# piotrmwojcik/GI-GS

Measured on AMD Instinct MI355X. Metric: train-step renders/sec (fwd+bwd, G-buffer+indirect) at 800x800; PSNR vs the CPU oracle, higher is better.
Workload: dtype f32; 1 GPU; C2 (configs[1] TensoIR lego stand-in): 300k surface Gaussians, 800x800, SH deg 2, GI step=16 start=8 delta=0.0625; P=300000, N=640000, M=9, hip_graphs=on, fused_glue=on, gi_march=proj, rasterizer=whole step = 2 hand-captured hipGraphs (fwd, bwd), asynchronous binning

## Files before the change

gi-gs_amd/csrc/api.hip:

```cpp
#include <cstdarg>
#include <cstdio>
#include <cstdlib>
#include <cstring>
#include <map>
#include <algorithm>
#include <new>
#include <mutex>
#include <vector>

#include "../../include/gigs_hip.h"
#include "gigs_common.h"

namespace {

thread_local char g_err[512] = "";

int fail(int code, const char* fmt, ...) {
  va_list ap;
  va_start(ap, fmt);
  vsnprintf(g_err, sizeof(g_err), fmt, ap);
  va_end(ap);
  return code;
}

// ... 38 lines not shown
  uint32_t step = msb;
  while (step > 1) {
    step /= 2;
    if (n >> msb) msb += step;
    else msb -= step;
  }
  if (n >> msb) msb++;
  return msb;
}

enum Stage {
  kPreprocess = 0, kScan, kDuplicate, kSort, kRanges, kBlendFwd, kBlendBwd, kPreprocessBwd,
  kDepthToNormal, kSsao, kSsr, kMedian, kBilateral, kMedianBwd, kShadeFwd, kShadeBwd,
  kCubemapFwd, kCubemapBwd, kGbufferPost, kLossFwd, kLossBwd, kL1SsimFwd, kL1SsimBwd, kTvFwd, kTvBwd,
  kMaskedL1, kAdam, kDensifyStats, kGatherRows, kDist2, kActivateFwd, kActivateBwd, kNumStages
};
const char* kStageNames[kNumStages] = {
  "preprocess_fwd", "scan", "duplicate", "sort", "tile_ranges", "blend_fwd", "blend_bwd",
  "preprocess_bwd", "depth_to_normal", "ssao", "ssr", "median3x3", "bilateral3x3",
  "median3x3_bwd", "shade_fwd", "shade_bwd", "cubemap_fwd", "cubemap_bwd", "gbuffer_post",
  "stage2_loss_fwd", "stage2_loss_bwd", "l1_ssim_fwd", "l1_ssim_bwd", "tv_loss_fwd", "tv_loss_bwd", "masked_l1",
  "adam_step", "densify_stats", "gather_rows", "dist2", "activate_fwd", "activate_bwd"};

int env_int(const char* name, int dflt) {
  const char* e = getenv(name);
  return (e && e[0]) ? atoi(e) : dflt;
}
gigs::Options options_from_env() {
  gigs::Options o;
  const char* b = getenv("GIGS_BINNING");
  o.binning_legacy = (b && strcmp(b, "legacy") == 0) ? 1 : 0;
  o.bucket_max_mean = env_int("GIGS_BUCKET_MAX_MEAN", gigs::kBucketMaxMeanList);
  const char* ll = getenv("GIGS_LONG_LISTS");
  o.long_lists = (ll && ll[0]) ? (ll[0] == '1' ? 1 : 0) : -1;
  o.bucket_target = std::max(256, env_int("GIGS_BUCKET_TARGET", 1536));
  o.bin_bands = std::max(0, env_int("GIGS_BIN_BANDS", 0));
  o.blend_cull = env_int("GIGS_BLEND_CULL", 1) != 0;
  o.pre_bwd_sh_skip = env_int("GIGS_PRE_BWD_SH_SKIP", 1) != 0;
  o.gi_march = 4;
  if (const char* e = getenv("GIGS_GI_MARCH")) {
    static const char* names[] = {"exact", "hoist", "hoist_fma", "proj_nr", "proj"};
    for (int i = 0; i < 5; i++)
      if (strcmp(e, names[i]) == 0) o.gi_march = i;
  }
  o.gi_cert = env_int("GIGS_GI_CERT", 1) != 0;
  o.gi_interleave = env_int("GIGS_GI_INTERLEAVE", 1) != 0;
  o.gi_tile_log2w = env_int("GIGS_GI_TILE_LOG2W", 3);
  if (o.gi_tile_log2w < 0 || o.gi_tile_log2w > 6) o.gi_tile_log2w = 3;
  o.gi_zero_rays = env_int("GIGS_GI_ZERO_RAYS", 0) != 0;
  o.spec_max8 = env_int("GIGS_SPEC_MAX8", 128);
  o.spec_max16 = env_int("GIGS_SPEC_MAX16", 1500);
  o.shade_lds_floats = env_int("GIGS_SHADE_LDS_FLOATS", 30 * 1024);
  o.shade_bwd_blocks = std::max(0, env_int("GIGS_SHADE_BWD_BLOCKS", 0));
  return o;
}
const gigs::Ctx& ctx_of(const gigs_ctx* c) { return c ? *reinterpret_cast<const gigs::Ctx*>(c) : gigs::default_ctx(); }

struct ProfRec { int stage; hipEvent_t a, b; };
std::mutex g_prof_mu;
bool g_prof_on = false;
std::vector<ProfRec> g_prof_recs;
std::vector<hipEvent_t> g_prof_pool;

hipEvent_t prof_event() {
  if (!g_prof_pool.empty()) {
    hipEvent_t e = g_prof_pool.back();
    g_prof_pool.pop_back();
    return e;
  }
  hipEvent_t e;
  hipEventCreate(&e);
  return e;
}

struct StageScope {
  hipStream_t s;
  int stage;
  bool on;
  hipEvent_t a, b;
  StageScope(int stage_, hipStream_t s_) : s(s_), stage(stage_), on(false) {
    std::lock_guard<std::mutex> lk(g_prof_mu);
    if (!g_prof_on) return;
    on = true;
    a = prof_event();
    b = prof_event();
    hipEventRecord(a, s);
  }
  ~StageScope() {
    if (!on) return;
    hipEventRecord(b, s);
    std::lock_guard<std::mutex> lk(g_prof_mu);
    g_prof_recs.push_back({stage, a, b});
  }
};

}

namespace gigs {
const Options& default_options() {
  static const Options o = options_from_env();
  return o;
}
const Ctx& default_ctx() {
  static const Ctx c = {default_options(), 0u, nullptr, nullptr, 0, nullptr, nullptr};
  return c;
}
// ... 21 lines not shown
  const size_t N = (size_t)width * height;
  const size_t T = (size_t)((width + GIGS_BLOCK_X - 1) / GIGS_BLOCK_X) * ((height + GIGS_BLOCK_Y - 1) / GIGS_BLOCK_Y);
  return gigs::required_bytes<gigs::ImageState>(N, T);
}
size_t gigs_required_binning(int R) {
  if (R < 0) { fail(GIGS_ERR_INVALID, "R < 0"); return 0; }
  return gigs::required_bytes<gigs::BinningState>((size_t)R, sort_size_cached(R));
}

long long gigs_geom_offset(int P, int which) {
  char* base = nullptr;
  char* p = base;
  gigs::GeomState g = gigs::GeomState::fromChunk(p, (size_t)P, 0);
  const void* ptrs[] = {g.depths, g.pos_view, g.means2D, g.cov3D, g.conic_opacity, g.rgb,
                        g.clamped, g.tiles_touched, g.point_offsets, g.internal_radii, g.brec, g.grec};
  if (which < 0 || which >= (int)(sizeof(ptrs) / sizeof(ptrs[0]))) return -1;
  return (long long)((const char*)ptrs[which] - base);
}
long long gigs_binning_offset(int R, int which) {
  char* base = nullptr;
  char* p = base;
  gigs::BinningState b = gigs::BinningState::fromChunk(p, (size_t)R, 0);
  const void* ptrs[] = {b.keys_unsorted, b.values_unsorted, b.keys, b.point_list, b.hit_mask};
  if (which < 0 || which >= 5) return -1;
  return (long long)((const char*)ptrs[which] - base);
}
long long gigs_image_offset(int width, int height, int which) {
  const size_t N = (size_t)width * height;
  const size_t T = (size_t)((width + GIGS_BLOCK_X - 1) / GIGS_BLOCK_X) * ((height + GIGS_BLOCK_Y - 1) / GIGS_BLOCK_Y);
  char* base = nullptr;
  char* p = base;
  gigs::ImageState s = gigs::ImageState::fromChunk(p, N, T);
  const void* ptrs[] = {s.final_T, s.n_contrib, s.ranges, s.tile_order};
  if (which < 0 || which >= 4) return -1;
  return (long long)((const char*)ptrs[which] - base);
}

gigs_ctx* gigs_ctx_create(void) {
  gigs::Ctx* c = new (std::nothrow) gigs::Ctx(gigs::default_ctx());
  if (!c) fail(GIGS_ERR_ALLOC, "gigs_ctx_create: out of host memory");
  return reinterpret_cast<gigs_ctx*>(c);
}
void gigs_ctx_destroy(gigs_ctx* ctx) { delete reinterpret_cast<gigs::Ctx*>(ctx); }

int gigs_ctx_get_options(const gigs_ctx* ctx, gigs_options* out) {
  if (!out || out->struct_bytes < (int)sizeof(gigs_options)) return fail(GIGS_ERR_INVALID, "gigs_ctx_get_options: set struct_bytes = sizeof(gigs_options)");
  const gigs::Options& o = ctx_of(ctx).opt;
  out->struct_bytes = (int)sizeof(gigs_options);
  out->binning_legacy = o.binning_legacy; out->bucket_max_mean = o.bucket_max_mean; out->long_lists = o.long_lists;
  out->bucket_target = o.bucket_target; out->bin_bands = o.bin_bands; out->blend_cull = o.blend_cull; out->pre_bwd_sh_skip = o.pre_bwd_sh_skip;
  out->gi_march = o.gi_march; out->gi_cert = o.gi_cert; out->gi_interleave = o.gi_interleave;
  out->gi_tile_log2w = o.gi_tile_log2w; out->gi_zero_rays = o.gi_zero_rays; out->spec_max8 = o.spec_max8;
  out->spec_max16 = o.spec_max16; out->shade_lds_floats = o.shade_lds_floats; out->shade_bwd_blocks = o.shade_bwd_blocks;
  return 0;
}
int gigs_ctx_set_options(gigs_ctx* ctx, const gigs_options* in) {
  if (!ctx) return fail(GIGS_ERR_INVALID, "gigs_ctx_set_options: the default context is immutable, create one");
  if (!in || in->struct_bytes < (int)sizeof(gigs_options)) return fail(GIGS_ERR_INVALID, "gigs_ctx_set_options: set struct_bytes = sizeof(gigs_options)");
  if (in->gi_march < 0 || in->gi_march > 4) return fail(GIGS_ERR_INVALID, "gi_march must be 0..4");
  if (in->gi_tile_log2w < 0 || in->gi_tile_log2w > 6) return fail(GIGS_ERR_INVALID, "gi_tile_log2w must be 0..6");
  if (in->long_lists < -1 || in->long_lists > 1) return fail(GIGS_ERR_INVALID, "long_lists must be -1, 0 or 1");
  if (in->bucket_target < 256 || in->bucket_max_mean < 0 || in->bin_bands < 0 || in->bin_bands > 64)
    return fail(GIGS_ERR_INVALID, "bucket_target >= 256, bucket_max_mean >= 0, 0 <= bin_bands <= 64");
  if (in->spec_max8 < 0 || in->spec_max16 < in->spec_max8) return fail(GIGS_ERR_INVALID, "0 <= spec_max8 <= spec_max16");
  if (in->shade_lds_floats < 0 || in->shade_bwd_blocks < 0) return fail(GIGS_ERR_INVALID, "shade_lds_floats, shade_bwd_blocks >= 0");
  gigs::Options& o = reinterpret_cast<gigs::Ctx*>(ctx)->opt;
  o.binning_legacy = in->binning_legacy != 0; o.bucket_max_mean = in->bucket_max_mean; o.long_lists = in->long_lists;
  o.bucket_target = in->bucket_target; o.bin_bands = in->bin_bands; o.blend_cull = in->blend_cull != 0; o.pre_bwd_sh_skip = in->pre_bwd_sh_skip != 0;
  o.gi_march = in->gi_march; o.gi_cert = in->gi_cert != 0; o.gi_interleave = in->gi_interleave != 0;
  o.gi_tile_log2w = in->gi_tile_log2w; o.gi_zero_rays = in->gi_zero_rays != 0; o.spec_max8 = in->spec_max8;
  o.spec_max16 = in->spec_max16; o.shade_lds_floats = in->shade_lds_floats; o.shade_bwd_blocks = in->shade_bwd_blocks;
  return 0;
}
int gigs_ctx_set_reuse_binning(gigs_ctx* ctx, int on) {
  if (!ctx) return fail(GIGS_ERR_INVALID, "gigs_ctx_set_reuse_binning: the default context is immutable, create one");
  reinterpret_cast<gigs::Ctx*>(ctx)->reuse_binning = on != 0;
  return 0;
}
int gigs_ctx_set_split_sh(gigs_ctx* ctx, const float* sh_rest) {
  if (!ctx) return fail(GIGS_ERR_INVALID, "gigs_ctx_set_split_sh: the default context is immutable, create one");
  reinterpret_cast<gigs::Ctx*>(ctx)->sh_rest = sh_rest;
  return 0;
}
int gigs_ctx_set_materials_only(gigs_ctx* ctx, void* violations) {
  if (!ctx) return fail(GIGS_ERR_INVALID, "gigs_ctx_set_materials_only: the default context is immutable, create one");
  reinterpret_cast<gigs::Ctx*>(ctx)->materials_only = reinterpret_cast<unsigned*>(violations);
  return 0;
}
int gigs_ctx_set_blend_begin_event(gigs_ctx* ctx, void* hip_event) {
  if (!ctx) return fail(GIGS_ERR_INVALID, "gigs_ctx_set_blend_begin_event: the default context is immutable, create one");
  reinterpret_cast<gigs::Ctx*>(ctx)->blend_begin_event = hip_event;
  return 0;
}

__global__ void __launch_bounds__(64) stream_delay_kernel(unsigned ticks) {
  const unsigned long long t0 = wall_clock64();
  while (wall_clock64() - t0 < (unsigned long long)ticks) __builtin_amdgcn_s_sleep(8);
}

int gigs_stream_delay(unsigned nanoseconds, void* stream) {
  if (nanoseconds == 0) return 0;
  const unsigned ns = nanoseconds > 1000000u ? 1000000u : nanoseconds;
  hipLaunchKernelGGL(stream_delay_kernel, dim3(1), dim3(64), 0, (hipStream_t)stream, (ns + 9u) / 10u);
  return hipGetLastError() == hipSuccess ? 0 : gigs_internal_fail(GIGS_ERR_HIP, "stream_delay: launch failed");
}

int gigs_ctx_set_async_binning(gigs_ctx* ctx, int r_capacity, unsigned* device_counters) {
  if (!ctx) return fail(GIGS_ERR_INVALID, "gigs_ctx_set_async_binning: the default context is immutable, create one");
  gigs::Ctx* c = reinterpret_cast<gigs::Ctx*>(ctx);
  c->async_capacity = r_capacity > 0 ? (unsigned)r_capacity : 0u;
  c->async_counters = r_capacity > 0 ? device_counters : nullptr;
  return 0;
}

void gigs_profile_begin(void) {
  std::lock_guard<std::mutex> lk(g_prof_mu);
  for (auto& r : g_prof_recs) { g_prof_pool.push_back(r.a); g_prof_pool.push_back(r.b); }
  g_prof_recs.clear();
  g_prof_on = true;
}

int gigs_profile_end(float* total_ms, int* launches, int n) {
  std::vector<ProfRec> recs;
  {
// ... 469 lines not shown
```

gi-gs_amd/csrc/gigs_common.h:

```cpp
#pragma once
#include <hip/hip_runtime.h>
#include <stdint.h>

#define GIGS_BLOCK_X 16
#define GIGS_BLOCK_Y 16
#define GIGS_TILE (GIGS_BLOCK_X * GIGS_BLOCK_Y)
#define GIGS_BREC_F4 5
#define GIGS_GREC 20

namespace gigs {

struct v3 { float x, y, z; };
struct v4 { float x, y, z, w; };

__device__ __forceinline__ v3 operator+(v3 a, v3 b) { return {a.x + b.x, a.y + b.y, a.z + b.z}; }
__device__ __forceinline__ v3 operator-(v3 a, v3 b) { return {a.x - b.x, a.y - b.y, a.z - b.z}; }
__device__ __forceinline__ v3 operator*(v3 a, float s) { return {a.x * s, a.y * s, a.z * s}; }
__device__ __forceinline__ float dot3(v3 a, v3 b) { return a.x * b.x + a.y * b.y + a.z * b.z; }
__device__ __forceinline__ v3 cross3(v3 a, v3 b) {
  return {a.y * b.z - a.z * b.y, a.z * b.x - a.x * b.z, a.x * b.y - a.y * b.x};
}
__device__ __forceinline__ v3 normalize3(v3 v) {
  float inv = 1.0f / sqrtf(dot3(v, v));
  return v * inv;
// ... 131 lines not shown
    carve(chunk, s.n_contrib, N);
    carve(chunk, s.ranges, T);
    carve(chunk, s.tile_order, T);
    carve(chunk, s.bin_hist, (size_t)(kBinGroups + 2) * T);
    carve(chunk, s.bin_counters, 4);
    return s;
  }
};

struct BinningState {
  uint64_t* keys_unsorted;
  uint32_t* values_unsorted;
  uint64_t* keys;
  uint32_t* point_list;
  uint8_t* hit_mask;
  char* sort_space;
  size_t sort_size;
  static BinningState fromChunk(char*& chunk, size_t R, size_t sort_size) {
    BinningState b;
    carve(chunk, b.keys_unsorted, R);
    carve(chunk, b.values_unsorted, R);
    carve(chunk, b.keys, R);
    carve(chunk, b.point_list, R);
    carve(chunk, b.hit_mask, 4 * R);
    b.sort_size = sort_size;
    carve(chunk, b.sort_space, sort_size);
    return b;
  }
};

template <typename S, typename... A>
inline size_t required_bytes(A... a) {
  char* p = nullptr;
  S::fromChunk(p, a...);
  return reinterpret_cast<size_t>(p) + kAlign;
}

struct Options {
  int binning_legacy;
  int bucket_max_mean;
  int long_lists;
  int bucket_target;
  int bin_bands;
  int blend_cull;
  int pre_bwd_sh_skip;
  int gi_march;
  int gi_cert;
  int gi_interleave;
  int gi_tile_log2w;
  int gi_zero_rays;
  int spec_max8, spec_max16;
  int shade_lds_floats;
  int shade_bwd_blocks;
};
struct Ctx {
  Options opt;
  unsigned async_capacity;
  unsigned* async_counters;
  void* blend_begin_event;
  int reuse_binning;
  unsigned* materials_only;
  const float* sh_rest;
};
const Options& default_options();
const Ctx& default_ctx();

struct FwdArgs {
  int P, D, M, W, H;
  unsigned gx, gy;
  float focal_x, focal_y, tan_fovx, tan_fovy, scale_modifier;
  const float *means3D, *shs, *colors_precomp, *opacities, *normal, *albedo, *roughness,
      *metallic, *scales, *rotations, *cov3D_precomp, *viewmatrix, *projmatrix, *cam_pos,
      *background;
  int argmax_depth, inference;
  const float* shs_rest;
};

void launch_preprocess_fwd(const FwdArgs& a, const GeomState& g, int* radii, hipStream_t s);
void launch_zero_words(uint32_t* p, size_t n, hipStream_t s);
void launch_bin_count(int P, const int* radii, unsigned gx, unsigned gy, const GeomState& g, const ImageState& img, hipStream_t s);
void launch_bin_prefix(int P, int T, unsigned capacity, const ImageState& img, unsigned* user_counters, hipStream_t s);
void launch_bin_scatter(int P, const int* radii, unsigned gx, unsigned gy, unsigned capacity, unsigned bands, const GeomState& g,
                        const BinningState& b, const ImageState& img, hipStream_t s);
int launch_bin_sort(int T, int P, bool long_lists, unsigned bucket_target, unsigned capacity, const BinningState& b, const ImageState& img,
                    hipStream_t s);
size_t long_space_bytes(size_t T, size_t R);
void launch_mark_visible(int P, const float* means3D, const float* viewmatrix, uint8_t* present,
                         hipStream_t s);
hipError_t scan_tiles(const GeomState& g, int P, hipStream_t s);
size_t scan_temp_bytes(int P);
size_t sort_temp_bytes(int R);
void launch_duplicate(int P, const int* radii, unsigned gx, unsigned gy, const GeomState& g,
                      const BinningState& b, hipStream_t s);
hipError_t sort_pairs(const BinningState& b, int R, int end_bit, hipStream_t s);
void launch_tile_ranges(int R, const BinningState& b, uint2* ranges, hipStream_t s);
void launch_tile_order(int T, const uint2* ranges, uint32_t* tile_order, hipStream_t s);
void launch_blend_fwd(const FwdArgs& a, const GeomState& g, const BinningState& b,
                      const ImageState& im, float* out_color, float* out_opacity,
                      float* out_depth, float* out_normal, float* out_normal_view, float* out_pos,
                      float* out_albedo, float* out_roughness, float* out_metallic, int cull, size_t hit_stride,
                      hipStream_t s, bool reused_lists = false);

struct BwdArgs {
  int P, D, M, R, W, H;
  unsigned gx, gy;
  float focal_x, focal_y, tan_fovx, tan_fovy, scale_modifier;
// ... 42 lines not shown
```

gi-gs_amd/csrc/pbr.hip:

```cpp
#include <cmath>
#include <cstdlib>
#include <cstring>
#include <map>
#include <mutex>
#include <vector>

#include "gigs_common.h"
#include "pixel_ops.h"

namespace gigs {

__device__ __forceinline__ v3 safe_normalize(v3 v) {
  const float l = sqrtf(v.x * v.x + v.y * v.y + v.z * v.z);
  return l > 0.0f ? v3{v.x / l, v.y / l, v.z / l} : v3{0, 0, 0};
}
__device__ __forceinline__ v3 cube_dir_raw(float fx, float fy, int side) {
  switch (side) {
    case 0: return {1, -fy, -fx};
    case 1: return {-1, -fy, fx};
    case 2: return {fx, 1, fy};
    case 3: return {fx, -1, -fy};
    case 4: return {fx, -fy, 1};
    default: return {-fx, -fy, -1};
  }
// ... 872 lines not shown
cube_taps_export_kernel(int res, int n, const float* __restrict__ dirs, int* __restrict__ idx, float* __restrict__ w) {
  const int i = blockIdx.x * 256 + threadIdx.x;
  if (i >= n) return;
  Taps t;
  const bool ok = cube_taps(res, dirs[3 * (size_t)i], dirs[3 * (size_t)i + 1], dirs[3 * (size_t)i + 2], t);
#pragma unroll
  for (int k = 0; k < 4; k++) {
    const bool use = ok && t.idx[k] >= 0 && t.w[k] != 0.0f;
    idx[4 * (size_t)i + k] = use ? t.idx[k] : -1;
    w[4 * (size_t)i + k] = use ? t.w[k] : 0.0f;
  }
}

__global__ void __launch_bounds__(256)
cube_texture_bwd_gather_kernel(int n_tex, const int* __restrict__ offsets, const int* __restrict__ ent_sample,
                               const float* __restrict__ ent_w, const float* __restrict__ g_out, int n, int planar,
                               float* __restrict__ d_tex, int heavy, int light_blocks, const int* __restrict__ heavy_ids,
                               int n_heavy) {
  auto grad = [&](int s, float& a, float& b, float& c) {
    if (planar) { a = g_out[s]; b = g_out[(size_t)n + s]; c = g_out[2 * (size_t)n + s]; }
    else { a = g_out[3 * (size_t)s]; b = g_out[3 * (size_t)s + 1]; c = g_out[3 * (size_t)s + 2]; }
  };
  if ((int)blockIdx.x < light_blocks) {
    const int t = blockIdx.x * 256 + threadIdx.x;
    if (t >= n_tex) return;
    const int b = offsets[t], e = offsets[t + 1];
    if (e - b > heavy) return;
    float c0 = 0.0f, c1 = 0.0f, c2 = 0.0f;
    for (int k = b; k < e; k++) {
      float g0, g1, g2;
      grad(ent_sample[k], g0, g1, g2);
      const float w = ent_w[k];
      c0 += g0 * w; c1 += g1 * w; c2 += g2 * w;
    }
    d_tex[3 * (size_t)t] = c0; d_tex[3 * (size_t)t + 1] = c1; d_tex[3 * (size_t)t + 2] = c2;
    return;
  }
  const int h = ((int)blockIdx.x - light_blocks) * 4 + (threadIdx.x >> 6);
  if (h >= n_heavy) return;
  const int lane = threadIdx.x & 63;
  const int t = heavy_ids[h];
  const int b = offsets[t], e = offsets[t + 1];
  float c0 = 0.0f, c1 = 0.0f, c2 = 0.0f;
  for (int k = b + lane; k < e; k += 64) {
    float g0, g1, g2;
    grad(ent_sample[k], g0, g1, g2);
    const float w = ent_w[k];
    c0 += g0 * w; c1 += g1 * w; c2 += g2 * w;
  }
  c0 = wave_sum63(c0); c1 = wave_sum63(c1); c2 = wave_sum63(c2);
  if (lane == 63) { d_tex[3 * (size_t)t] = c0; d_tex[3 * (size_t)t + 1] = c1; d_tex[3 * (size_t)t + 2] = c2; }
}

__global__ void __launch_bounds__(kShadeBwdBlock)
shade_bwd_kernel(ShadeArgs A) {
  extern __shared__ __align__(16) float s_lds[];
  for (int i = threadIdx.x; i < A.lds_total; i += kShadeBwdBlock) s_lds[i] = 0.0f;
  __syncthreads();
  const int n_chunks = (A.H * A.W + kShadeBwdBlock - 1) / kShadeBwdBlock;
  for (int chunk = blockIdx.x; chunk < n_chunks; chunk += gridDim.x) {
  const int pg = chunk * kShadeBwdBlock + threadIdx.x;
  const bool live = pg < A.H * A.W;
  const int p = live ? pg : 0;
  ShadePix q;
  shade_pixel(A, p, q);
  float g_dl[3] = {0, 0, 0}, g_sp[3] = {0, 0, 0};
  if (live) {
    const bool mk = A.mask[p] != 0;
    const size_t e = (size_t)p * A.ps, cs = A.cs;
    const float gscale = A.g_scale ? A.g_scale[0] : 1.0f;
    float g_d[3] = {0, 0, 0}, g_s[3] = {0, 0, 0};
    const float pre_d[3] = {q.drgb.x, q.drgb.y, q.drgb.z}, pre_s[3] = {q.srgb.x, q.srgb.y, q.srgb.z};
#pragma unroll
    for (int c = 0; c < 3; c++) {
      float g = (A.g_render && mk) ? A.g_render[e + c * cs] * gscale : 0.0f;
      if (g != 0.0f) {
        float x = pre_d[c] + pre_s[c], d_tone = 1.0f, d_gam = 1.0f;
        if (A.tone) x = aces(x, d_tone);
        const float xc = fminf(fmaxf(x, 0.0f), 1.0f);
        const float d_clamp = (x >= 0.0f && x <= 1.0f) ? 1.0f : 0.0f;
        if (A.gamma) lin2srgb(xc, d_gam);
        g = g * d_gam * d_clamp * d_tone;
      }
      float gd = A.g_diffuse_rgb ? A.g_diffuse_rgb[e + c * cs] : 0.0f;
      float gs = A.g_specular_rgb ? A.g_specular_rgb[e + c * cs] : 0.0f;
      if (A.gamma) {
        float d1, d2;
        lin2srgb(pre_d[c], d1);
        lin2srgb(pre_s[c], d2);
        gd *= d1;
        gs *= d2;
      }
      g_d[c] = g + gd;
      g_s[c] = g + gs;
    }
    const float av[3] = {q.a.x, q.a.y, q.a.z}, dlv[3] = {q.dl.x, q.dl.y, q.dl.z};
    const float spv[3] = {q.sp.x, q.sp.y, q.sp.z}, F0v[3] = {q.F0.x, q.F0.y, q.F0.z};
    const float reflv[3] = {q.refl.x, q.refl.y, q.refl.z};
    const float s0v[3] = {q.s0.x, q.s0.y, q.s0.z}, s1v[3] = {q.s1.x, q.s1.y, q.s1.z};
    float d_alb[3], d_m = 0.0f, d_fgx = 0.0f, d_fgy = 0.0f, d_lvl = 0.0f;
#pragma unroll
    for (int c = 0; c < 3; c++) {
      d_alb[c] = g_d[c] * dlv[c];
      g_dl[c] = g_d[c] * av[c] + (A.g_diffuse_light ? A.g_diffuse_light[e + c * cs] : 0.0f);
      g_sp[c] = g_s[c] * reflv[c];
      const float g_refl = g_s[c] * spv[c];
      const float dF0 = g_refl * q.fgx;
      d_fgx += g_refl * F0v[c];
      d_fgy += g_refl;
      if (A.metallic) {
        d_m += dF0 * (av[c] - 0.04f);
        d_alb[c] += dF0 * q.m;
      }
      if (q.l1 != q.l0) d_lvl += g_sp[c] * (s1v[c] - s0v[c]);
    }
#pragma unroll
    for (int c = 0; c < 3; c++) {
      if (A.g_albedo_mul_a) d_alb[c] += (A.g_albedo_mul_a[e + c * cs] * gscale) * A.g_albedo_mul_b[e + c * cs];
      A.d_albedo[e + c * cs] = d_alb[c];
    }
    float add_r = A.g_roughness_add ? A.g_roughness_add[p] : 0.0f, add_m = A.g_metallic_add ? A.g_metallic_add[p] : 0.0f;
    if (A.lamb_mask) {
      const float m = A.lamb_mask[p], cnt = A.lamb_acc4[3];
      add_r += -m / cnt * (0.001f * gscale);
      add_m += m / cnt * (0.001f * gscale);
    }
    if (A.d_metallic) A.d_metallic[p] = d_m + add_m;
    const float d_r = d_fgx * q.dfgx_dv + d_fgy * q.dfgy_dv + (q.lvl_inside ? d_lvl * q.dmdr : 0.0f);
    A.d_roughness[p] = (d_r + add_r) * A.rough_scale;
  }
#ifdef GIGS_DIAG
#define GIGS_ABLATED(bit) (A.ablate & (bit))
#else
#define GIGS_ABLATED(bit) 0
#endif
  if (A.d_diffuse && !GIGS_ABLATED(1)) {
    float* base = A.lds_diffuse_off >= 0 ? s_lds + A.lds_diffuse_off : A.d_diffuse;
#pragma unroll
    for (int k = 0; k < 4; k++) {
      const int idx = (live && q.has_d) ? q.td.idx[k] : -1;
      const float w = idx >= 0 ? q.td.w[k] * q.occ : 0.0f;
      run_add3<false>(base + 3 * (size_t)max(idx, 0), idx, g_dl[0] * w, g_dl[1] * w, g_dl[2] * w);
    }
  }
  if (!GIGS_ABLATED(2)) {
    const float wl = (q.l1 != q.l0) ? (1 - q.lf) : 1.0f;
    float* t0 = A.lds_spec_off[q.l0] >= 0 ? s_lds + A.lds_spec_off[q.l0] : A.d_spec[q.l0];
    float* t1 = A.lds_spec_off[q.l1] >= 0 ? s_lds + A.lds_spec_off[q.l1] : A.d_spec[q.l1];
    if (!A.d_spec[q.l0]) t0 = nullptr;
    if (!A.d_spec[q.l1]) t1 = nullptr;
#ifdef GIGS_DIAG
    if (((A.ablate & 4) && A.lds_spec_off[q.l0] >= 0) || ((A.ablate & 8) && A.lds_spec_off[q.l0] < 0)) t0 = nullptr;
    if (((A.ablate & 4) && A.lds_spec_off[q.l1] >= 0) || ((A.ablate & 8) && A.lds_spec_off[q.l1] < 0)) t1 = nullptr;
#endif
#pragma unroll
    for (int k = 0; k < 4; k++) {
      const int idx = (live && q.has0 && t0) ? q.t0.idx[k] : -1;
      const float w = idx >= 0 ? q.t0.w[k] * wl : 0.0f;
      run_add3<false>(t0 ? t0 + 3 * (size_t)max(idx, 0) : nullptr, idx >= 0 ? (q.l0 << 24) | idx : -1, g_sp[0] * w, g_sp[1] * w, g_sp[2] * w);
    }
#pragma unroll
    for (int k = 0; k < 4; k++) {
      const int idx = (live && q.l1 != q.l0 && q.has1 && t1) ? q.t1.idx[k] : -1;
      const float w = idx >= 0 ? q.t1.w[k] * q.lf : 0.0f;
      run_add3<false>(t1 ? t1 + 3 * (size_t)max(idx, 0) : nullptr, idx >= 0 ? (q.l1 << 24) | idx : -1, g_sp[0] * w, g_sp[1] * w, g_sp[2] * w);
    }
  }
  }
  if (A.lds_total > 0) {
    __syncthreads();
    if (A.lds_diffuse_off >= 0 && A.d_diffuse) {
      const int n = 6 * A.diffuse_res * A.diffuse_res * 3;
      for (int i = threadIdx.x; i < n; i += kShadeBwdBlock) {
        const float val = s_lds[A.lds_diffuse_off + i];
        if (val != 0.0f) atomicAdd(A.d_diffuse + i, val);
      }
    }
    for (int l = 0; l < A.L; l++) {
      if (A.lds_spec_off[l] < 0 || !A.d_spec[l]) continue;
      const int n = 6 * A.spec_res[l] * A.spec_res[l] * 3;
      for (int i = threadIdx.x; i < n; i += kShadeBwdBlock) {
        const float val = s_lds[A.lds_spec_off[l] + i];
        if (val != 0.0f) atomicAdd(A.d_spec[l] + i, val);
      }
    }
  }
}

}

#include "../../include/gigs_hip.h"

extern "C" {

int gigs_internal_fail(int code, const char* msg);
void gigs_internal_stage_begin(int stage, void* stream, void** token);
void gigs_internal_stage_end(void* token);
const gigs::Options* gigs_internal_options(const gigs_ctx* ctx);

#define PBR_CHECK_LAUNCH()                                        \
  do {                                                            \
    if (hipGetLastError() != hipSuccess) return gigs_internal_fail(GIGS_ERR_HIP, "pbr kernel launch failed"); \
  } while (0)

int gigs_diffuse_cubemap_fwd(int res, const float* cubemap, float* out, void* stream) {
  if (res <= 0 || !cubemap || !out) return gigs_internal_fail(GIGS_ERR_INVALID, "diffuse_cubemap_fwd: bad argument");
  hipStream_t s = (hipStream_t)stream;
  const float4* table = gigs::texel_table(res, s);
  if (!table) return gigs_internal_fail(GIGS_ERR_HIP, "texel table");
  void* tok; gigs_internal_stage_begin(16, stream, &tok);
  hipLaunchKernelGGL(gigs::diffuse_cubemap_kernel<false>, dim3((6 * res * res + 3) / 4), dim3(256), 0, s, res, table, cubemap, out);
  gigs_internal_stage_end(tok);
  PBR_CHECK_LAUNCH();
  return 0;
}

int gigs_diffuse_cubemap_bwd(int res, const float* grad_out, float* grad_cubemap, void* stream) {
  if (res <= 0 || !grad_out || !grad_cubemap) return gigs_internal_fail(GIGS_ERR_INVALID, "diffuse_cubemap_bwd: bad argument");
// ... 330 lines not shown
  }
  A.ps = 1; A.cs = H * W;
  A.render_rgb = render_rgb; A.out_linear = out_linear;
  void* tok; gigs_internal_stage_begin(14, stream, &tok);
  hipLaunchKernelGGL(gigs::shade_fwd_multi_kernel, dim3((H * W + 255) / 256), dim3(256), 0, (hipStream_t)stream, A, Ls);
  gigs_internal_stage_end(tok);
  PBR_CHECK_LAUNCH();
  return 0;
}

int gigs_shade_bwd(int H, int W, const float* normals, const float* view_dirs, const float* albedo,
                   const float* roughness, const uint8_t* mask, const float* occlusion,
                   const float* metallic, const float* diffuse, int diffuse_res, int n_levels,
                   const float* const* spec, const int* spec_res, const float* lut, int lut_w, int lut_h,
                   int tone, int gamma, const float* g_render, const float* g_diffuse_rgb,
                   const float* g_specular_rgb, const float* g_diffuse_light, float* d_albedo,
                   float* d_roughness, float* d_metallic, float* d_diffuse, float* const* d_spec,
                   void* stream) {
  return gigs_shade_bwd_ex(nullptr, H, W, normals, view_dirs, albedo, roughness, mask, occlusion, metallic, diffuse, diffuse_res,
                           n_levels, spec, spec_res, lut, lut_w, lut_h, tone, gamma, g_render, g_diffuse_rgb,
                           g_specular_rgb, g_diffuse_light, d_albedo, d_roughness, d_metallic, d_diffuse, d_spec, nullptr,
                           stream);
}

int gigs_shade_bwd_ex(gigs_ctx* ctx, int H, int W, const float* normals, const float* view_dirs, const float* albedo,
                      const float* roughness, const uint8_t* mask, const float* occlusion,
                      const float* metallic, const float* diffuse, int diffuse_res, int n_levels,
                      const float* const* spec, const int* spec_res, const float* lut, int lut_w, int lut_h,
                      int tone, int gamma, const float* g_render, const float* g_diffuse_rgb,
                      const float* g_specular_rgb, const float* g_diffuse_light, float* d_albedo,
                      float* d_roughness, float* d_metallic, float* d_diffuse, float* const* d_spec,
                      const gigs_shade_ext* ext, void* stream) {
  gigs::ShadeArgs A;
  const int rc = fill_shade(A, H, W, normals, view_dirs, albedo, roughness, mask, occlusion, metallic, nullptr,
                            diffuse, diffuse_res, n_levels, spec, spec_res, lut, lut_w, lut_h, tone, gamma);
  if (rc) return rc;
  if (apply_shade_ext(A, ext, true)) return GIGS_ERR_INVALID;
  if (!d_albedo || !d_roughness) return gigs_internal_fail(GIGS_ERR_INVALID, "shade_bwd: null output");
  A.g_render = g_render; A.g_diffuse_rgb = g_diffuse_rgb; A.g_specular_rgb = g_specular_rgb; A.g_diffuse_light = g_diffuse_light;
  A.d_albedo = d_albedo; A.d_roughness = d_roughness; A.d_metallic = d_metallic; A.d_diffuse = d_diffuse;
  for (int i = 0; i < n_levels; i++) A.d_spec[i] = d_spec ? d_spec[i] : nullptr;
  int used = 0;
  A.lds_diffuse_off = -1;
  for (int i = 0; i < 8; i++) A.lds_spec_off[i] = -1;
  const int n_dd = 6 * diffuse_res * diffuse_res * 3;
  const gigs::Options& o = *gigs_internal_options(ctx);
  const int lds_budget = o.shade_lds_floats < 0 ? 0 : (o.shade_lds_floats > gigs::kShadeLdsBudget ? gigs::kShadeLdsBudget : o.shade_lds_floats);
  if (d_diffuse && n_dd <= lds_budget) { A.lds_diffuse_off = 0; used = n_dd; }
  for (int i = n_levels - 1; i >= 0; i--) {
    const int n = 6 * spec_res[i] * spec_res[i] * 3;
    if (A.d_spec[i] && used + n <= lds_budget) { A.lds_spec_off[i] = used; used += n; }
  }
  A.lds_total = used;
  static bool attr_set = false;
  if (!attr_set) {
    if (hipFuncSetAttribute(reinterpret_cast<const void*>(gigs::shade_bwd_kernel), hipFuncAttributeMaxDynamicSharedMemorySize,
                            gigs::kShadeLdsBudget * (int)sizeof(float)) != hipSuccess)
      return gigs_internal_fail(GIGS_ERR_HIP, "shade_bwd: cannot raise the dynamic LDS limit");
    attr_set = true;
  }
  void* tok; gigs_internal_stage_begin(15, stream, &tok);
  const int n_chunks = (H * W + gigs::kShadeBwdBlock - 1) / gigs::kShadeBwdBlock;
  static const int n_cus = [] {
    int dev = 0, cus = 256;
    if (hipGetDevice(&dev) == hipSuccess) hipDeviceGetAttribute(&cus, hipDeviceAttributeMultiprocessorCount, dev);
    return cus;
  }();
  const int max_blocks = o.shade_bwd_blocks > 0 ? o.shade_bwd_blocks : n_cus;
  const int blocks = (n_chunks < max_blocks) ? n_chunks : max_blocks;
  hipLaunchKernelGGL(gigs::shade_bwd_kernel, dim3(blocks), dim3(gigs::kShadeBwdBlock), (size_t)used * sizeof(float),
                     (hipStream_t)stream, A);
  gigs_internal_stage_end(tok);
  PBR_CHECK_LAUNCH();
  return 0;
}

}
```

gi-gs_amd/gigs_lib.py:

```python
from __future__ import annotations

import ctypes as C
import functools
import os
import threading

_HERE = os.path.dirname(os.path.abspath(__file__))
LIB_PATH = os.environ.get("GIGS_LIB", os.path.join(_HERE, "libgigs_hip.so"))

ALLOC_FN = C.CFUNCTYPE(C.c_void_p, C.c_size_t, C.c_void_p)

_f = C.c_void_p
_i = C.c_int
_fl = C.c_float

SIGNATURES = {
    "gigs_last_error": (C.c_char_p, []),
    "gigs_build_arch": (C.c_char_p, []),
    "gigs_required_geom": (C.c_size_t, [_i]),
    "gigs_required_image": (C.c_size_t, [_i, _i]),
    "gigs_required_binning": (C.c_size_t, [_i]),
    "gigs_forward": (_i, [C.c_void_p, ALLOC_FN, C.c_void_p, ALLOC_FN, C.c_void_p, ALLOC_FN, C.c_void_p,
                          _i, _i, _i, _f, _i, _i,
                          _f, _f, _f, _f, _f, _f, _f, _f,
# ... 83 lines not shown
    "gigs_normal_angular_error": (_i, [_i, _i, _f, _f, _i, _f, _f, _f, C.c_void_p]),
    "gigs_lpips_vgg_weight_floats": (C.c_size_t, []),
    "gigs_lpips_vgg_pack": (_i, [C.POINTER(C.c_void_p), C.POINTER(C.c_void_p), C.POINTER(C.c_void_p), _f, C.c_void_p]),
    "gigs_lpips_vgg_scratch_bytes": (C.c_size_t, [_i, _i, _i]),
    "gigs_lpips_vgg": (_i, [_i, _i, _i, _f, _f, _i, _f, _f, _f, _f, C.POINTER(C.c_void_p), C.c_void_p]),
    "gigs_tv_loss_fwd": (_i, [_i, _i, _i, _i, _f, _f, _f, _f, _f, C.c_void_p]),
    "gigs_tv_loss_bwd": (_i, [_i, _i, _i, _i, _f, _f, _f, _f, _f, C.c_void_p]),
    "gigs_masked_l1_fwd": (_i, [_i, _i, _i, _f, _f, _f, _f, _f, C.c_void_p]),
    "gigs_masked_l1_bwd": (_i, [_i, _i, _i, _f, _f, _f, _f, _f, _f, _f, C.c_void_p]),
    "gigs_adam_step": (_i, [_i, C.c_void_p, C.c_double, C.c_double, C.c_double, _i, C.c_void_p]),
    "gigs_adam_step_dyn": (_i, [_i, C.c_void_p, C.c_double, C.c_double, C.c_double, _i, _f, C.c_void_p]),
    "gigs_adam_scalars": (None, [C.c_double, _i, C.c_double, C.c_double, C.POINTER(C.c_float)]),
    "gigs_adam_step_watch": (_i, [_i, C.c_void_p, C.c_double, C.c_double, C.c_double, _i, _f, C.c_char_p, _f, C.c_void_p]),
    "gigs_adam_step_guarded": (_i, [_i, C.c_void_p, C.c_double, C.c_double, C.c_double, _i, _f, C.c_char_p, _f, _f, C.c_void_p]),
    "gigs_ctx_set_reuse_binning": (_i, [C.c_void_p, _i]),
    "gigs_ctx_set_materials_only": (_i, [C.c_void_p, C.c_void_p]),
    "gigs_ctx_set_split_sh": (_i, [C.c_void_p, C.c_void_p]),
    "gigs_activate_fwd": (_i, [_i, _i, C.c_void_p, C.c_void_p, C.c_void_p]),
    "gigs_activate_bwd": (_i, [_i, _i, C.c_void_p, C.c_void_p, C.c_void_p, C.c_void_p]),
    "gigs_densify_stats": (_i, [_i, _f, _f, _f, _f, _f, _f, _f, C.c_void_p]),
    "gigs_densify_stats_guarded": (_i, [_i, _f, _f, _f, _f, _f, _f, _f, _f, C.c_void_p]),
    "gigs_gather_rows": (_i, [_i, C.c_void_p, C.c_longlong, C.c_longlong, _f, _f, C.c_void_p]),
    "gigs_dist2_scratch_bytes": (C.c_size_t, [_i]),
    "gigs_dist2": (_i, [_i, _f, _f, _f, C.c_size_t, C.c_void_p]),
    "gigs_geom_offset": (C.c_longlong, [_i, _i]),
    "gigs_binning_offset": (C.c_longlong, [_i, _i]),
    "gigs_image_offset": (C.c_longlong, [_i, _i, _i]),
    "gigs_selftest_div2": (_i, [_i, _f, _f, _f, _f, _f, _f, C.c_void_p]),
    "gigs_selftest_round": (_i, [_f, C.c_void_p]),
    "gigs_ctx_set_blend_begin_event": (_i, [C.c_void_p, C.c_void_p]),
    "gigs_stream_delay": (_i, [C.c_uint, C.c_void_p]),
    "gigs_ctx_set_async_binning": (_i, [C.c_void_p, _i, C.c_void_p]),
    "gigs_ctx_create": (C.c_void_p, []),
    "gigs_ctx_destroy": (None, [C.c_void_p]),
    "gigs_ctx_get_options": (_i, [C.c_void_p, C.c_void_p]),
    "gigs_ctx_set_options": (_i, [C.c_void_p, C.c_void_p]),
    "gigs_profile_begin": (None, []),
    "gigs_profile_end": (_i, [C.POINTER(C.c_float), C.POINTER(C.c_int), _i]),
    "gigs_profile_stage_name": (C.c_char_p, [_i]),
}

class ShadeExt(C.Structure):
    _fields_ = [("planar", C.c_int), ("rough_scale", C.c_float), ("rough_bias", C.c_float),
                ("out_F0", C.c_void_p), ("out_linear", C.c_void_p), ("out_roughness", C.c_void_p),
                ("g_albedo_mul_a", C.c_void_p), ("g_albedo_mul_b", C.c_void_p),
                ("g_roughness_add", C.c_void_p), ("g_metallic_add", C.c_void_p),
                ("g_scale", C.c_void_p), ("lamb_mask", C.c_void_p), ("lamb_acc4", C.c_void_p)]


class Options(C.Structure):
    _fields_ = [(n, C.c_int) for n in (
        "struct_bytes", "binning_legacy", "bucket_max_mean", "long_lists", "bucket_target", "bin_bands", "blend_cull",
        "pre_bwd_sh_skip", "gi_march", "gi_cert", "gi_interleave", "gi_tile_log2w", "gi_zero_rays", "spec_max8",
        "spec_max16", "shade_lds_floats", "shade_bwd_blocks")]


OPTION_NAMES = tuple(n for n, _ in Options._fields_ if n != "struct_bytes")
GI_MARCHES = ("exact", "hoist", "hoist_fma", "proj_nr", "proj")


class SpecLevel(C.Structure):
    _fields_ = [("res", C.c_int), ("avg_window", C.c_int), ("src", C.c_void_p), ("bounds", C.c_void_p),
                ("offsets", C.c_void_p), ("weights", C.c_void_p), ("dst", C.c_void_p), ("wsum", C.c_void_p)]


class AdamGroup(C.Structure):
    _fields_ = [("param", C.c_void_p), ("grad", C.c_void_p), ("exp_avg", C.c_void_p), ("exp_avg_sq", C.c_void_p),
                ("n", C.c_longlong), ("lr", C.c_double), ("step", C.c_int)]


class ActivationRaw(C.Structure):
    _fields_ = [(n, C.c_void_p) for n in ("f_dc", "f_rest", "opacity", "normal", "albedo", "roughness", "metallic",
                                          "scaling", "rotation")]


class ActivationOut(C.Structure):
    _fields_ = [(n, C.c_void_p) for n in ("shs", "opacities", "normal", "albedo", "roughness", "metallic", "scales",
                                          "rotations")]


class GatherTensor(C.Structure):
    _fields_ = [("src", C.c_void_p), ("dst", C.c_void_p), ("row_floats", C.c_int), ("zero_new", C.c_int)]


_lib = None


class GigsError(RuntimeError):
    pass


def lib():
    global _lib
    if _lib is None:
        if not os.path.exists(LIB_PATH):
            raise ImportError(
                f"{LIB_PATH} not found: build it with `python gi-gs_amd/build.py` "
                "(hipcc, --offload-arch=gfx950). There is no CPU fallback.")
        l = C.CDLL(LIB_PATH)
        for name, (res, args) in SIGNATURES.items():
            fn = getattr(l, name)
            fn.restype = res
            fn.argtypes = args
        _lib = l
    return _lib


# ... 174 lines not shown
```

include/gigs_hip.h:

```cpp
#ifndef GIGS_HIP_H_
#define GIGS_HIP_H_

#include <stddef.h>
#include <stdint.h>

#ifdef __cplusplus
extern "C" {
#endif

#define GIGS_OK 0
#define GIGS_ERR_INVALID (-1)
#define GIGS_ERR_HIP (-2)
#define GIGS_ERR_ALLOC (-3)

typedef char* (*gigs_alloc_fn)(size_t nbytes, void* user);

const char* gigs_last_error(void);
const char* gigs_build_arch(void);

typedef struct gigs_ctx gigs_ctx;
typedef struct gigs_options {
  int struct_bytes;
  int binning_legacy;
  int bucket_max_mean;
  int long_lists;
  int bucket_target;
  int bin_bands;
  int blend_cull;
  int pre_bwd_sh_skip;
  int gi_march;
  int gi_cert;
  int gi_interleave;
  int gi_tile_log2w;
  int gi_zero_rays;
  int spec_max8;
  int spec_max16;
  int shade_lds_floats;
  int shade_bwd_blocks;
} gigs_options;
gigs_ctx* gigs_ctx_create(void);
void gigs_ctx_destroy(gigs_ctx* ctx);
int gigs_ctx_get_options(const gigs_ctx* ctx, gigs_options* out);
int gigs_ctx_set_options(gigs_ctx* ctx, const gigs_options* in);

size_t gigs_required_geom(int P);
size_t gigs_required_image(int width, int height);
size_t gigs_required_binning(int num_rendered);

int gigs_forward(gigs_ctx* ctx, gigs_alloc_fn geometryBuffer, void* geom_user, gigs_alloc_fn binningBuffer,
                 void* binning_user, gigs_alloc_fn imageBuffer, void* image_user, int P, int D, int M,
                 const float* background, int width, int height, const float* means3D,
                 const float* shs, const float* colors_precomp, const float* opacities,
                 const float* normal, const float* albedo, const float* roughness,
                 const float* metallic, const float* scales, float scale_modifier,
                 const float* rotations, const float* cov3D_precomp, const float* viewmatrix,
                 const float* projmatrix, const float* cam_pos, float tan_fovx, float tan_fovy,
                 int prefiltered, int argmax_depth, int inference, float* out_color,
                 float* out_opacity, float* out_depth, float* out_normal, float* out_normal_view,
                 float* out_pos, float* out_albedo, float* out_roughness, float* out_metallic,
                 int* radii, int debug, void* stream);

int gigs_backward(gigs_ctx* ctx, int P, int D, int M, int R, const float* background, int width, int height,
                  const float* means3D, const float* shs, const float* colors_precomp,
                  const float* normal, const float* albedo, const float* roughness,
                  const float* metallic, const float* scales, const float* rotations,
                  const float* cov3D_precomp, const float* viewmatrix, const float* projmatrix,
                  const float* cam_pos, const int* radii, float scale_modifier, float tan_fovx,
                  float tan_fovy, char* geom_buffer, char* binning_buffer, char* image_buffer,
                  const float* dL_dpix_depth, const float* dL_dpix, const float* dL_dpix_opacity,
                  const float* dL_dpix_normal, const float* dL_dpix_albedo,
                  const float* dL_dpix_roughness, const float* dL_dpix_metallic, float* dL_dmean2D,
                  float* dL_dconic, float* dL_ddepth, float* dL_dopacity, float* dL_dnormal,
                  float* dL_dalbedo, float* dL_droughness, float* dL_dmetallic, float* dL_dcolor,
                  float* dL_dmean3D, float* dL_dcov3D, float* dL_dsh, float* dL_dscale,
                  float* dL_drot, int debug, void* stream);

int gigs_mark_visible(int P, const float* means3D, const float* viewmatrix,
                      const float* projmatrix, uint8_t* present, void* stream);

int gigs_depth_to_normal(int width, int height, float focal_x, float focal_y,
                         const float* viewmatrix, const float* depth, float* normal,
                         float* depth_pos, void* stream);

int gigs_derive_normal(int width, int height, float focal_x, float focal_y, const float* viewmatrix, const float* depth,
                       float sigma_color, float sigma_x, float sigma_y, float* normal_from_depth, float* depth_pos_filter,
                       void* stream);
int gigs_ssao(int width, int height, float focal_x, float focal_y, float radius, float bias,
              float thick, float delta, int step, int start, const float* normal_view,
              const float* pos, float* occlusion, void* stream);

int gigs_ssr(int width, int height, float focal_x, float focal_y, float radius, float bias,
// ... 261 lines not shown
```

Before: 333.1 renders/s.

## Use 2D pixel tiles and wave-level key dedup in shading backward

The shading backward kernel now maps each 256-thread block to a 32x32 pixel tile, with each wave covering an 8x8 sub-tile instead of a row-linear chunk. Neighbouring pixels in a wave are more likely to hit the same specular texels. For texels held in global memory, a wave-level dedup loop reduces identical keys across lanes and issues one atomic per unique texel, with a fallback run-add after a fixed number of rounds. This aims to cut global atomic contention, at the cost of extra ballot and reduction work and less coalesced pixel access. The old row layout stays available behind a new option.

Result: faster. 343.4 renders/s, median of 6 (+3.1%).

```diff
diff --git a/gi-gs_amd/csrc/api.hip b/gi-gs_amd/csrc/api.hip
--- a/gi-gs_amd/csrc/api.hip
+++ b/gi-gs_amd/csrc/api.hip
@@ -114,6 +114,7 @@
   o.spec_max16 = env_int("GIGS_SPEC_MAX16", 1500);
   o.shade_lds_floats = env_int("GIGS_SHADE_LDS_FLOATS", 30 * 1024);
   o.shade_bwd_blocks = std::max(0, env_int("GIGS_SHADE_BWD_BLOCKS", 0));
+  o.shade_bwd_rows = env_int("GIGS_SHADE_BWD_ROWS", 0) != 0;
   return o;
 }
 const gigs::Ctx& ctx_of(const gigs_ctx* c) { return c ? *reinterpret_cast<const gigs::Ctx*>(c) : gigs::default_ctx(); }
@@ -241,6 +242,7 @@
   out->gi_march = o.gi_march; out->gi_cert = o.gi_cert; out->gi_interleave = o.gi_interleave;
   out->gi_tile_log2w = o.gi_tile_log2w; out->gi_zero_rays = o.gi_zero_rays; out->spec_max8 = o.spec_max8;
   out->spec_max16 = o.spec_max16; out->shade_lds_floats = o.shade_lds_floats; out->shade_bwd_blocks = o.shade_bwd_blocks;
+  out->shade_bwd_rows = o.shade_bwd_rows;
   return 0;
 }
 int gigs_ctx_set_options(gigs_ctx* ctx, const gigs_options* in) {
@@ -259,6 +261,7 @@
   o.gi_march = in->gi_march; o.gi_cert = in->gi_cert != 0; o.gi_interleave = in->gi_interleave != 0;
   o.gi_tile_log2w = in->gi_tile_log2w; o.gi_zero_rays = in->gi_zero_rays != 0; o.spec_max8 = in->spec_max8;
   o.spec_max16 = in->spec_max16; o.shade_lds_floats = in->shade_lds_floats; o.shade_bwd_blocks = in->shade_bwd_blocks;
+  o.shade_bwd_rows = in->shade_bwd_rows != 0;
   return 0;
 }
 int gigs_ctx_set_reuse_binning(gigs_ctx* ctx, int on) {
diff --git a/gi-gs_amd/csrc/gigs_common.h b/gi-gs_amd/csrc/gigs_common.h
--- a/gi-gs_amd/csrc/gigs_common.h
+++ b/gi-gs_amd/csrc/gigs_common.h
@@ -207,6 +207,7 @@
   int spec_max8, spec_max16;
   int shade_lds_floats;
   int shade_bwd_blocks;
+  int shade_bwd_rows;
 };
 struct Ctx {
   Options opt;
diff --git a/gi-gs_amd/csrc/pbr.hip b/gi-gs_amd/csrc/pbr.hip
--- a/gi-gs_amd/csrc/pbr.hip
+++ b/gi-gs_amd/csrc/pbr.hip
@@ -948,15 +948,61 @@
   if (lane == 63) { d_tex[3 * (size_t)t] = c0; d_tex[3 * (size_t)t + 1] = c1; d_tex[3 * (size_t)t + 2] = c2; }
 }
 
+constexpr int kWaveDedupRounds = 24;
+__device__ __forceinline__ void wave_dedup_add(float* const (&d_spec)[8], int (&key)[8], const float (&v)[8][3]) {
+  const int lane = threadIdx.x & 63;
+  for (int round = 0; round < kWaveDedupRounds; round++) {
+    int first = -1;
+#pragma unroll
+    for (int k = 7; k >= 0; k--) first = key[k] >= 0 ? key[k] : first;
+    const unsigned long long pend = __builtin_amdgcn_ballot_w64(first >= 0);
+    if (pend == 0ull) return;
+    const int K = __builtin_amdgcn_readlane(first, (int)__builtin_ctzll(pend));
+    float s0 = 0.0f, s1 = 0.0f, s2 = 0.0f;
+#pragma unroll
+    for (int k = 0; k < 8; k++) {
+      const bool m = key[k] == K;
+      s0 += m ? v[k][0] : 0.0f;
+      s1 += m ? v[k][1] : 0.0f;
+      s2 += m ? v[k][2] : 0.0f;
+      key[k] = m ? -1 : key[k];
+    }
+    s0 = wave_sum63(s0); s1 = wave_sum63(s1); s2 = wave_sum63(s2);
+    const float c0 = __int_as_float(__builtin_amdgcn_readlane(__float_as_int(s0), 63));
+    const float c1 = __int_as_float(__builtin_amdgcn_readlane(__float_as_int(s1), 63));
+    const float c2 = __int_as_float(__builtin_amdgcn_readlane(__float_as_int(s2), 63));
+    const float s = lane == 0 ? c0 : (lane == 1 ? c1 : c2);
+    if (lane < 3 && s != 0.0f) atomicAdd(d_spec[K >> 24] + 3 * (size_t)(K & 0xffffff) + lane, s);
+  }
+#pragma unroll
+  for (int k = 0; k < 8; k++) {
+    if (__builtin_amdgcn_ballot_w64(key[k] >= 0) == 0ull) continue;
+    float* t = key[k] >= 0 ? d_spec[key[k] >> 24] + 3 * (size_t)(key[k] & 0xffffff) : nullptr;
+    run_add3<false>(t, key[k], v[k][0], v[k][1], v[k][2]);
+  }
+}
+
+template <bool kTiles>
 __global__ void __launch_bounds__(kShadeBwdBlock)
 shade_bwd_kernel(ShadeArgs A) {
   extern __shared__ __align__(16) float s_lds[];
   for (int i = threadIdx.x; i < A.lds_total; i += kShadeBwdBlock) s_lds[i] = 0.0f;
   __syncthreads();
-  const int n_chunks = (A.H * A.W + kShadeBwdBlock - 1) / kShadeBwdBlock;
+  const int tiles_x = (A.W + 31) / 32;
+  const int n_chunks = kTiles ? tiles_x * ((A.H + 31) / 32) : (A.H * A.W + kShadeBwdBlock - 1) / kShadeBwdBlock;
   for (int chunk = blockIdx.x; chunk < n_chunks; chunk += gridDim.x) {
-  const int pg = chunk * kShadeBwdBlock + threadIdx.x;
-  const bool live = pg < A.H * A.W;
+  int pg;
+  bool live;
+  if (kTiles) {
+    const int wv = threadIdx.x >> 6, ln = threadIdx.x & 63;
+    const int x = (chunk % tiles_x) * 32 + (wv & 3) * 8 + (ln & 7);
+    const int y = (chunk / tiles_x) * 32 + (wv >> 2) * 8 + (ln >> 3);
+    live = x < A.W && y < A.H;
+    pg = y * A.W + x;
+  } else {
+    pg = chunk * kShadeBwdBlock + threadIdx.x;
+    live = pg < A.H * A.W;
+  }
   const int p = live ? pg : 0;
   ShadePix q;
   shade_pixel(A, p, q);
@@ -1049,6 +1095,27 @@
     if (((A.ablate & 4) && A.lds_spec_off[q.l0] >= 0) || ((A.ablate & 8) && A.lds_spec_off[q.l0] < 0)) t0 = nullptr;
     if (((A.ablate & 4) && A.lds_spec_off[q.l1] >= 0) || ((A.ablate & 8) && A.lds_spec_off[q.l1] < 0)) t1 = nullptr;
 #endif
+    if (kTiles) {
+      const bool glob0 = A.lds_spec_off[q.l0] < 0, glob1 = A.lds_spec_off[q.l1] < 0;
+      int gkey[8];
+      float gv[8][3];
+#pragma unroll
+      for (int k = 0; k < 8; k++) {
+        const bool first = k < 4;
+        const int idx = first ? ((live && q.has0 && t0) ? q.t0.idx[k] : -1)
+                              : ((live && q.l1 != q.l0 && q.has1 && t1) ? q.t1.idx[k - 4] : -1);
+        const float w = idx >= 0 ? (first ? q.t0.w[k] * wl : q.t1.w[k - 4] * q.lf) : 0.0f;
+        const float v0 = g_sp[0] * w, v1 = g_sp[1] * w, v2 = g_sp[2] * w;
+        const int key = idx >= 0 ? ((first ? q.l0 : q.l1) << 24) | idx : -1;
+        const bool glob = first ? glob0 : glob1;
+        gkey[k] = (glob && (v0 != 0.0f || v1 != 0.0f || v2 != 0.0f)) ? key : -1;
+        gv[k][0] = v0; gv[k][1] = v1; gv[k][2] = v2;
+        const int lkey = glob ? -1 : key;
+        if (__builtin_amdgcn_ballot_w64(lkey >= 0) != 0ull)
+          run_add3<false>(lkey >= 0 ? (first ? t0 : t1) + 3 * (size_t)idx : nullptr, lkey, v0, v1, v2);
+      }
+      wave_dedup_add(A.d_spec, gkey, gv);
+    } else {
 #pragma unroll
     for (int k = 0; k < 4; k++) {
       const int idx = (live && q.has0 && t0) ? q.t0.idx[k] : -1;
@@ -1060,6 +1127,7 @@
       const int idx = (live && q.l1 != q.l0 && q.has1 && t1) ? q.t1.idx[k] : -1;
       const float w = idx >= 0 ? q.t1.w[k] * q.lf : 0.0f;
       run_add3<false>(t1 ? t1 + 3 * (size_t)max(idx, 0) : nullptr, idx >= 0 ? (q.l1 << 24) | idx : -1, g_sp[0] * w, g_sp[1] * w, g_sp[2] * w);
+    }
     }
   }
   }
@@ -1496,15 +1564,17 @@
     if (A.d_spec[i] && used + n <= lds_budget) { A.lds_spec_off[i] = used; used += n; }
   }
   A.lds_total = used;
-  static bool attr_set = false;
-  if (!attr_set) {
-    if (hipFuncSetAttribute(reinterpret_cast<const void*>(gigs::shade_bwd_kernel), hipFuncAttributeMaxDynamicSharedMemorySize,
-                            gigs::kShadeLdsBudget * (int)sizeof(float)) != hipSuccess)
+  const bool rows = o.shade_bwd_rows != 0;
+  const void* fn = rows ? reinterpret_cast<const void*>(gigs::shade_bwd_kernel<false>)
+                        : reinterpret_cast<const void*>(gigs::shade_bwd_kernel<true>);
+  static bool attr_set[2] = {false, false};
+  if (!attr_set[rows]) {
+    if (hipFuncSetAttribute(fn, hipFuncAttributeMaxDynamicSharedMemorySize, gigs::kShadeLdsBudget * (int)sizeof(float)) != hipSuccess)
       return gigs_internal_fail(GIGS_ERR_HIP, "shade_bwd: cannot raise the dynamic LDS limit");
-    attr_set = true;
+    attr_set[rows] = true;
   }
   void* tok; gigs_internal_stage_begin(15, stream, &tok);
-  const int n_chunks = (H * W + gigs::kShadeBwdBlock - 1) / gigs::kShadeBwdBlock;
+  const int n_chunks = rows ? (H * W + gigs::kShadeBwdBlock - 1) / gigs::kShadeBwdBlock : ((W + 31) / 32) * ((H + 31) / 32);
   static const int n_cus = [] {
     int dev = 0, cus = 256;
     if (hipGetDevice(&dev) == hipSuccess) hipDeviceGetAttribute(&cus, hipDeviceAttributeMultiprocessorCount, dev);
@@ -1512,11 +1582,15 @@
   }();
   const int max_blocks = o.shade_bwd_blocks > 0 ? o.shade_bwd_blocks : n_cus;
   const int blocks = (n_chunks < max_blocks) ? n_chunks : max_blocks;
-  hipLaunchKernelGGL(gigs::shade_bwd_kernel, dim3(blocks), dim3(gigs::kShadeBwdBlock), (size_t)used * sizeof(float),
-                     (hipStream_t)stream, A);
-  gigs_internal_stage_end(tok);
-  PBR_CHECK_LAUNCH();
-  return 0;
-}
-
-}
+  if (rows)
+    hipLaunchKernelGGL(gigs::shade_bwd_kernel<false>, dim3(blocks), dim3(gigs::kShadeBwdBlock), (size_t)used * sizeof(float),
+                       (hipStream_t)stream, A);
+  else
+    hipLaunchKernelGGL(gigs::shade_bwd_kernel<true>, dim3(blocks), dim3(gigs::kShadeBwdBlock), (size_t)used * sizeof(float),
+                       (hipStream_t)stream, A);
+  gigs_internal_stage_end(tok);
+  PBR_CHECK_LAUNCH();
+  return 0;
+}
+
+}
diff --git a/gi-gs_amd/gigs_lib.py b/gi-gs_amd/gigs_lib.py
--- a/gi-gs_amd/gigs_lib.py
+++ b/gi-gs_amd/gigs_lib.py
@@ -159,7 +159,7 @@
     _fields_ = [(n, C.c_int) for n in (
         "struct_bytes", "binning_legacy", "bucket_max_mean", "long_lists", "bucket_target", "bin_bands", "blend_cull",
         "pre_bwd_sh_skip", "gi_march", "gi_cert", "gi_interleave", "gi_tile_log2w", "gi_zero_rays", "spec_max8",
-        "spec_max16", "shade_lds_floats", "shade_bwd_blocks")]
+        "spec_max16", "shade_lds_floats", "shade_bwd_blocks", "shade_bwd_rows")]
 
 
 OPTION_NAMES = tuple(n for n, _ in Options._fields_ if n != "struct_bytes")
diff --git a/include/gigs_hip.h b/include/gigs_hip.h
--- a/include/gigs_hip.h
+++ b/include/gigs_hip.h
@@ -37,6 +37,7 @@
   int spec_max16;
   int shade_lds_floats;
   int shade_bwd_blocks;
+  int shade_bwd_rows;
 } gigs_options;
 gigs_ctx* gigs_ctx_create(void);
 void gigs_ctx_destroy(gigs_ctx* ctx);
```
